# ExaScience/elprep

Measured on AMD Instinct MI355X. Metric: Mreads/s through sort+markdup+BQSR, 150bp PE, higher is better.
Workload: dtype u8/int32/int64 (integer path; float64 finalize on host)

## Files before the change

elprep_amd/csrc/markdup.hip:

```cpp
#include "common.hpp"
#include "markdup_plan.hpp"

namespace elp {

constexpr uint32_t EMPTY = 0xFFFFFFFFu;
constexpr unsigned long long PB_EMPTY = ~0ull;

struct MdCols {
  uint64_t n;
  const int32_t *refid;
  const uint16_t *flag_in;
  const uint16_t *rgid;
  const uint16_t *rg_lib;
  const uint16_t *split;
  const int32_t *upos, *score;
  const uint64_t *qname_off;
  const uint8_t *qname;
};

__device__ __forceinline__ bool is_candidate(uint16_t f) { return (f & (F_UNMAPPED | F_SECONDARY | F_SUPPLEMENTARY)) == 0; }
__device__ __forceinline__ bool is_true_pair(uint16_t f) { return (f & (F_MULTIPLE | F_NEXT_UNMAPPED)) == F_MULTIPLE; }
__device__ __forceinline__ uint16_t lib_of(const MdCols &m, uint32_t i) {
  const uint16_t rg = m.rgid[i];
  return rg == ELP_NIL16 ? (uint16_t)ELP_NIL16 : m.rg_lib[rg];
}
__device__ __forceinline__ uint32_t ld_agent(const uint32_t *p) { return __hip_atomic_load(p, __ATOMIC_RELAXED, __HIP_MEMORY_SCOPE_AGENT); }
__device__ __forceinline__ unsigned long long ld_agent64(const unsigned long long *p) {
  return __hip_atomic_load(p, __ATOMIC_RELAXED, __HIP_MEMORY_SCOPE_AGENT);
}

__device__ __forceinline__ bool key_eq(const uint4 &a, const uint4 &b) { return a.x == b.x && a.y == b.y && a.z == b.z && a.w == b.w; }
__device__ __forceinline__ uint64_t frag_hash(const uint4 &k) {
  const uint64_t h = ((uint64_t)k.x << 32) | k.y;
  return mix64(mix64(h) ^ (((uint64_t)k.w << 32) | (uint64_t)k.z));
}

template <class Eq>
__device__ __forceinline__ uint32_t find_or_insert(uint32_t *table, uint64_t mask, uint64_t h, uint32_t i, Eq eq, uint64_t limit = ~0ull) {
  uint64_t s = h & mask;
  for (uint64_t probes = 0;; probes++) {
    if (probes > limit) return EMPTY;
    const uint32_t cur = atomicCAS(&table[s], EMPTY, i);
    if (cur == EMPTY) return i;
    if (cur == i || eq(cur, i)) return cur;
    s = (s + 1) & mask;
  }
}

__global__ __launch_bounds__(256) void k_frag_insert(MdCols m, const uint4 *__restrict__ fkey, const uint32_t *__restrict__ flist, uint32_t nf,
                                                     uint32_t *table, uint64_t mask, uint32_t *__restrict__ frep, unsigned long long *fbest) {
  const uint32_t j = blockIdx.x * blockDim.x + threadIdx.x;
  if (j >= nf) return;
  const uint32_t i = flist[j];
  const uint4 mine = fkey[i];
  const uint32_t rep = find_or_insert(table, mask, frag_hash(mine), i, [&](uint32_t a, uint32_t) { return key_eq(fkey[a], mine); });
  frep[i] = rep;
  atomicMax(&fbest[rep], (unsigned long long)(uint32_t)m.score[i]);
}
__global__ __launch_bounds__(256) void k_frag_bits(const uint32_t *__restrict__ table, uint64_t nwords, uint32_t *__restrict__ bits) {
  const uint64_t w = (uint64_t)blockIdx.x * blockDim.x + threadIdx.x;
  if (w >= nwords) return;
  const uint4 *t = reinterpret_cast<const uint4 *>(table + 32 * w);
  uint32_t b = 0;
#pragma unroll
  for (int k = 0; k < 8; k++) {
    const uint4 v = t[k];
    b |= (v.x != EMPTY ? 1u : 0u) << (4 * k) | (v.y != EMPTY ? 2u : 0u) << (4 * k) | (v.z != EMPTY ? 4u : 0u) << (4 * k) | (v.w != EMPTY ? 8u : 0u) << (4 * k);
  }
  bits[w] = b;
}
__device__ __forceinline__ void tournament(const MdCols &m, uint32_t *winner, uint32_t me) {
  uint32_t w = ld_agent(winner);
  for (;;) {
    if (w == EMPTY) {
      const uint32_t old = atomicCAS(winner, EMPTY, me);
      if (old == EMPTY) return;
      w = old;
      continue;
    }
    const int cq = qname_cmp(m.qname, m.qname_off, me, w);
    const bool better = cq < 0 || (cq == 0 && me > w);
    if (!better) return;
    const uint32_t old = atomicCAS(winner, w, me);
    if (old == w) return;
    w = old;
  }
}

__global__ __launch_bounds__(256) void k_frag_tie(MdCols m, const uint32_t *__restrict__ flist, uint32_t nf, const uint32_t *__restrict__ frep,
                                                  const unsigned long long *__restrict__ fbest, uint32_t *fwinner) {
  const uint32_t j = blockIdx.x * blockDim.x + threadIdx.x;
  if (j >= nf) return;
  const uint32_t i = flist[j];
  const uint32_t rep = frep[i];
  const unsigned long long b = fbest[rep];
  if ((b >> 63) || (unsigned long long)(uint32_t)m.score[i] != b) return;
  tournament(m, &fwinner[rep], (uint32_t)i);
}

__global__ __launch_bounds__(256) void k_frag_flag(MdCols m, const uint32_t *__restrict__ flist, uint32_t nf, const uint32_t *__restrict__ frep,
                                                   const unsigned long long *__restrict__ fbest, const uint32_t *__restrict__ fwinner,
                                                   uint16_t *__restrict__ flag_out) {
  const uint32_t j = blockIdx.x * blockDim.x + threadIdx.x;
  if (j >= nf) return;
  const uint32_t i = flist[j];
  const uint32_t rep = frep[i];
  const unsigned long long b = fbest[rep];
  const bool dup = (b >> 63) || (unsigned long long)(uint32_t)m.score[i] < b || fwinner[rep] != (uint32_t)i;
  if (dup) flag_out[i] = (uint16_t)(flag_out[i] | F_DUPLICATE);
}

struct PairKey { uint4 k1, k2; };
__device__ __forceinline__ PairKey pair_key(const uint4 &second, const uint4 &first) {
  const int32_t r1 = (int32_t)second.x, r2 = (int32_t)first.x, p1 = (int32_t)second.y, p2 = (int32_t)first.y;
  const bool v1 = second.z & 1u, v2 = first.z & 1u;
  const bool swap = r1 > r2 || (r1 == r2 && (p1 > p2 || (p1 == p2 && v1 && !v2)));
  return swap ? PairKey{first, second} : PairKey{second, first};
}
__device__ __forceinline__ bool pair_key_eq(const PairKey &a, const PairKey &b) {
  return a.k1.x == b.k1.x && a.k2.x == b.k2.x && a.k1.y == b.k1.y && a.k2.y == b.k2.y && a.k1.z == b.k1.z && ((a.k2.z ^ b.k2.z) & 1u) == 0 &&
         a.k1.w == b.k1.w;
}

__device__ __forceinline__ uint64_t pair_hash(const PairKey &k) {
  uint64_t h = mix64(((uint64_t)k.k1.x << 32) | k.k2.x);
  h = mix64(h ^ (((uint64_t)k.k1.y << 32) | k.k2.y));
  return mix64(h ^ (((uint64_t)k.k1.z << 1) | (k.k2.z & 1u)) ^ ((uint64_t)k.k1.w << 40));
}

__device__ __forceinline__ uint64_t qname_hash(const MdCols &m, uint32_t i) {
  const uint64_t o = m.qname_off[i];
  const uint32_t l = (uint32_t)(m.qname_off[i + 1] - o);
  uint64_t h = 0x9e3779b97f4a7c15ull ^ l;
  for (uint32_t k = 0; k < l; k += 8) h = (h ^ low_bytes(load8(m.qname + o + k), l - k)) * 0xff51afd7ed558ccdull + (h >> 29);
  return mix64(h ^ ((uint64_t)lib_of(m, i) << 48) ^ ((uint64_t)m.split[i] << 24));
}
__device__ __forceinline__ bool mate_key_eq(const MdCols &m, const uint4 *__restrict__ fkey, uint32_t a, const uint4 &kb, uint32_t b) {
  const uint4 ka = fkey[a];
  return (ka.z >> 1) == (kb.z >> 1) && ka.w == kb.w && qname_eq(m.qname, m.qname_off, a, b);
}
__device__ __forceinline__ bool is_mate_candidate(uint16_t f) { return is_candidate(f) && is_true_pair(f); }

enum : uint8_t { MC_NONE = 0, MC_TABLE = 1, MC_LEAD = 2, MC_FOLLOW = 3, MC_KIND = 3, MC_TABBED = 4  };
constexpr uint32_t MATE_BIG = 0xFFFFFFFEu;

__global__ __launch_bounds__(256) void k_bloom_coarse(const uint32_t *__restrict__ bloom, uint32_t n_lines, uint32_t *__restrict__ coarse) {
  const uint32_t line = blockIdx.x * 256 + threadIdx.x;
  bool nz = false;
  if (line < n_lines) {
    const uint4 *l = reinterpret_cast<const uint4 *>(bloom + (size_t)line * 16);
    const uint4 a = l[0], b = l[1], c2 = l[2], d = l[3];
    nz = (a.x | a.y | a.z | a.w | b.x | b.y | b.z | b.w | c2.x | c2.y | c2.z | c2.w | d.x | d.y | d.z | d.w) != 0;
  }
  const unsigned long long bits = __ballot(nz);
// ... 132 lines not shown
  if (i >= n) return;
  const uint32_t r = rep_of[i];
  if (r == EMPTY) return;
  uint32_t rep;
  if (r == MATE_BIG) rep = (uint32_t)i;
  else if (rep_of[r] == MATE_BIG) rep = r;
  else return;
  const uint32_t at = atomicAdd(count, 1u);
  keys[at] = ((uint64_t)rep << 32) | (uint64_t)i;
  vals[at] = (uint32_t)i;
  mate[i] = EMPTY;
}
__global__ __launch_bounds__(256) void k_big_pair(uint32_t cnt, const uint64_t *__restrict__ keys, uint32_t *mate) {
  const uint32_t j = blockIdx.x * 256 + threadIdx.x;
  if (j >= cnt) return;
  const uint32_t rep = (uint32_t)(keys[j] >> 32);
  if (j > 0 && (uint32_t)(keys[j - 1] >> 32) == rep) return;
  for (uint32_t k = j; k + 1 < cnt && (uint32_t)(keys[k + 1] >> 32) == rep; k += 2) {
    const uint32_t a = (uint32_t)keys[k], b = (uint32_t)keys[k + 1];
    mate[a] = b;
    mate[b] = a;
  }
}

__device__ __forceinline__ uint64_t pair_entry(const MdCols &m, const uint4 &later, const uint4 &earlier, uint32_t i, uint32_t mt) {
  return ((uint64_t)(uint32_t)(m.score[i] + m.score[mt]) << 32) | (uint32_t)pair_hash(pair_key(later, earlier));
}
__global__ __launch_bounds__(256) void k_pair_list_table(MdCols m, const uint4 *__restrict__ fkey, const uint32_t *__restrict__ mate,
                                                         const uint8_t *__restrict__ code, uint64_t *__restrict__ pk, uint32_t *__restrict__ pv,
                                                         uint32_t *np) {
  __shared__ uint64_t lk[PL_TILES * 256];
  __shared__ uint32_t lv[PL_TILES * 256];
  __shared__ uint32_t lcount, gbase;
  if (threadIdx.x == 0) lcount = 0;
  __syncthreads();
#pragma unroll 2
  for (int tile = 0; tile < PL_TILES; tile++) {
    const uint64_t i64 = ((uint64_t)blockIdx.x * PL_TILES + (uint64_t)tile) * 256 + threadIdx.x;
    const uint32_t i = (uint32_t)i64;
    const uint32_t mt = (i64 < m.n && (code[i64] & MC_TABBED)) ? mate[i] : EMPTY;
    const bool own = mt != EMPTY && mt < i;
    uint64_t key = 0;
    if (own) key = pair_entry(m, fkey[i], fkey[mt], i, mt);
    const unsigned long long mask = __ballot(own);
    if (mask) {
      const int lane = threadIdx.x & 63, leader = __ffsll((long long)mask) - 1;
      uint32_t at = 0;
      if (lane == leader) at = atomicAdd(&lcount, (uint32_t)__popcll(mask));
      at = __shfl(at, leader, 64);
      if (own) {
        at += (uint32_t)__popcll(mask & ((1ull << lane) - 1ull));
        lk[at] = key;
        lv[at] = i;
      }
    }
  }
  __syncthreads();
  if (threadIdx.x == 0) gbase = lcount ? atomicAdd(np, lcount) : 0u;
  __syncthreads();
  for (uint32_t k = threadIdx.x; k < lcount; k += 256) {
    pk[gbase + k] = lk[k];
    pv[gbase + k] = lv[k];
  }
}

__global__ __launch_bounds__(256) void k_pair_list_lists(MdCols m, const uint4 *__restrict__ fkey, const uint32_t *__restrict__ mate, const uint32_t *__restrict__ tab_list,
                                                         const uint32_t *__restrict__ tab_cnt, uint32_t cap, uint64_t *__restrict__ pk, uint32_t *__restrict__ pv, uint32_t *np) {
  __shared__ uint32_t first[65];
  if (threadIdx.x < 64) {
    uint32_t incl = tab_cnt[threadIdx.x * 16u];
    for (int d = 1; d < 64; d <<= 1) {
      const uint32_t up = __shfl_up(incl, d, 64);
      if ((int)threadIdx.x >= d) incl += up;
    }
    first[threadIdx.x + 1] = incl;
    if (threadIdx.x == 0) first[0] = 0;
  }
  __syncthreads();
  __shared__ uint64_t lk[PL_TILES * 256];
  __shared__ uint32_t lv[PL_TILES * 256];
  __shared__ uint32_t lcount, gbase;
  const uint32_t total = first[64], chunk = PL_TILES * 256u;
  for (uint32_t c0 = blockIdx.x * chunk; c0 < total; c0 += gridDim.x * chunk) {
    if (threadIdx.x == 0) lcount = 0;
    __syncthreads();
#pragma unroll 2
    for (int tile = 0; tile < PL_TILES; tile++) {
      const uint32_t g = c0 + (uint32_t)tile * 256u + threadIdx.x;
      uint32_t i = 0, mt = EMPTY;
      if (g < total) {
        uint32_t lo = 0, hi = 64;
        while (hi - lo > 1) {
          const uint32_t mid = (lo + hi) >> 1;
          if (first[mid] <= g) lo = mid; else hi = mid;
        }
        i = tab_list[(size_t)lo * cap + (g - first[lo])];
        mt = mate[i];
      }
      const bool own = mt != EMPTY && mt < i;
      uint64_t key = 0;
      if (own) key = pair_entry(m, fkey[i], fkey[mt], i, mt);
      const unsigned long long mask = __ballot(own);
      if (mask) {
        const int lane = threadIdx.x & 63, leader = __ffsll((long long)mask) - 1;
        uint32_t at = 0;
        if (lane == leader) at = atomicAdd(&lcount, (uint32_t)__popcll(mask));
        at = __shfl(at, leader, 64);
        if (own) {
          at += (uint32_t)__popcll(mask & ((1ull << lane) - 1ull));
          lk[at] = key;
          lv[at] = i;
        }
      }
    }
    __syncthreads();
    if (threadIdx.x == 0) gbase = lcount ? atomicAdd(np, lcount) : 0u;
    __syncthreads();
    for (uint32_t k = threadIdx.x; k < lcount; k += 256) {
      pk[gbase + k] = lk[k];
      pv[gbase + k] = lv[k];
    }
    __syncthreads();
  }
}

__device__ __forceinline__ uint32_t pair_bucket(uint64_t key, int sbits, int bbits) {
  return bbits ? ((uint32_t)key & ((1u << sbits) - 1u)) >> (sbits - bbits) : 0u;
}
__global__ __launch_bounds__(256) void k_pair_bounds(const uint64_t *__restrict__ ks, const uint32_t *__restrict__ np, int sbits, int bbits,
                                                     uint32_t *__restrict__ bstart, uint32_t *__restrict__ bend) {
  const uint32_t n = *np;
  const uint32_t j = blockIdx.x * 256 + threadIdx.x;
  if (j >= n) return;
  const uint32_t b = pair_bucket(ks[j], sbits, bbits);
  if (j == 0 || pair_bucket(ks[j - 1], sbits, bbits) != b) bstart[b] = j;
  if (j + 1 == n || pair_bucket(ks[j + 1], sbits, bbits) != b) bend[b] = j + 1;
}

__device__ __forceinline__ PairKey pair_key_of(const uint4 *__restrict__ fkey, const uint32_t *__restrict__ mate, uint32_t owner) {
  return pair_key(fkey[owner], fkey[mate[owner]]);
}
__device__ __forceinline__ void tournament_lds(const MdCols &m, uint32_t *winner, uint32_t me) {
  uint32_t w = *(volatile uint32_t *)winner;
  for (;;) {
    if (w != EMPTY) {
      const int cq = qname_cmp(m.qname, m.qname_off, me, w);
      if (!(cq < 0 || (cq == 0 && me > w))) return;
    }
    const uint32_t old = atomicCAS(winner, w, me);
    if (old == w) return;
    w = old;
  }
}
__device__ __forceinline__ void pair_lost(const MdCols &m, const uint32_t *__restrict__ mate, uint32_t o, uint32_t w, uint32_t *__restrict__ pair_win,
                                          uint16_t *__restrict__ flag_out) {
  const uint32_t mt = mate[o];
  pair_win[o] = w;
  flag_out[o] = (uint16_t)(flag_out[o] | F_DUPLICATE);
  flag_out[mt] = (uint16_t)(flag_out[mt] | F_DUPLICATE);
}

constexpr int PB_ECAP = 1024;

__device__ __forceinline__ int pb_slot(const MdCols &m, const uint4 *__restrict__ fkey, const uint32_t *__restrict__ mate,
                                       unsigned long long *s_key, uint32_t tmask, uint32_t h32, uint32_t o, bool insert) {
  uint32_t idx = (h32 * 0x9E3779B1u) >> 16 & tmask;
  const unsigned long long mine = ((unsigned long long)h32 << 32) | o;
  for (uint32_t probes = 0; probes <= tmask; probes++, idx = (idx + 1) & tmask) {
    unsigned long long cur = insert ? atomicCAS(&s_key[idx], PB_EMPTY, mine) : s_key[idx];
    if (cur == PB_EMPTY) { if (insert) return (int)idx; else continue; }
    if (cur == mine) return (int)idx;
    if ((uint32_t)(cur >> 32) == h32 && pair_key_eq(pair_key_of(fkey, mate, (uint32_t)cur), pair_key_of(fkey, mate, o))) return (int)idx;
  }
  return -1;
}

__global__ __launch_bounds__(PB_THREADS) void k_pair_bucket(MdCols m, const uint4 *__restrict__ fkey, const uint32_t *__restrict__ mate,
                                                     const uint64_t *__restrict__ ks, uint32_t *__restrict__ vs,
                                                     const uint32_t *__restrict__ bstart, const uint32_t *__restrict__ bend, int cap_slots,
                                                     uint32_t *__restrict__ pair_win, uint16_t *__restrict__ flag_out, int inv_end ) {
  __shared__ unsigned long long s_key[PB_CAP];
  __shared__ uint32_t s_best[PB_CAP], s_win[PB_CAP];
  __shared__ uint16_t s_slot[PB_ECAP];
  __shared__ uint32_t s_full, s_min, s_h;
  const uint32_t start = bstart[blockIdx.x], end = inv_end ? ~bend[blockIdx.x] : bend[blockIdx.x];
  if (end <= start) return;
  const uint32_t cnt = end - start;
  const uint32_t t = threadIdx.x;
  if (cnt == 1) return;
  uint32_t T = 2;
  while (T < 2 * cnt && T < (uint32_t)cap_slots) T <<= 1;
  const uint32_t tmask = T - 1;
  for (uint32_t k = t; k < T; k += PB_THREADS) { s_key[k] = PB_EMPTY; s_best[k] = 0; s_win[k] = EMPTY; }
  if (t == 0) s_full = 0;
  __syncthreads();
  ks += start;
  vs += start;
  for (uint32_t e = t; e < cnt; e += PB_THREADS) {
    const uint64_t key = ks[e];
    const uint32_t o = vs[e];
    if (o == EMPTY) continue;
    const int slot = pb_slot(m, fkey, mate, s_key, tmask, (uint32_t)key, o, true);
    if (slot < 0) { s_full = 1; break; }
    atomicMax(&s_best[slot], (uint32_t)(key >> 32));
    if (e < PB_ECAP) s_slot[e] = (uint16_t)slot;
  }
  __syncthreads();
  if (!s_full) {
    for (uint32_t e = t; e < cnt; e += PB_THREADS) {
      const uint64_t key = ks[e];
      const uint32_t o = vs[e];
      if (o == EMPTY) continue;
      const int slot = e < PB_ECAP ? (int)s_slot[e] : pb_slot(m, fkey, mate, s_key, tmask, (uint32_t)key, o, false);
      if ((uint32_t)(key >> 32) == s_best[slot]) tournament_lds(m, &s_win[slot], o);
    }
    __syncthreads();
    for (uint32_t e = t; e < cnt; e += PB_THREADS) {
      const uint32_t o = vs[e];
      if (o == EMPTY) continue;
      const int slot = e < PB_ECAP ? (int)s_slot[e] : pb_slot(m, fkey, mate, s_key, tmask, (uint32_t)ks[e], o, false);
      const uint32_t w = s_win[slot];
      if (w != o) pair_lost(m, mate, o, w, pair_win, flag_out);
    }
    return;
  }
  for (;;) {
    __syncthreads();
    if (t == 0) { s_min = EMPTY; s_best[0] = 0; s_win[0] = EMPTY; }
    __syncthreads();
    for (uint32_t e = t; e < cnt; e += PB_THREADS) {
      const uint32_t o = vs[e];
      if (o != EMPTY) atomicMin(&s_min, o);
    }
    __syncthreads();
    const uint32_t rep = s_min;
    if (rep == EMPTY) return;
    for (uint32_t e = t; e < cnt; e += PB_THREADS)
      if (vs[e] == rep) s_h = (uint32_t)ks[e];
    __syncthreads();
    const uint32_t rh = s_h;
    const PairKey rk = pair_key_of(fkey, mate, rep);
    for (uint32_t e = t; e < cnt; e += PB_THREADS) {
      const uint32_t o = vs[e];
      if (o != EMPTY && (uint32_t)ks[e] == rh && pair_key_eq(rk, pair_key_of(fkey, mate, o))) atomicMax(&s_best[0], (uint32_t)(ks[e] >> 32));
    }
    __syncthreads();
    for (uint32_t e = t; e < cnt; e += PB_THREADS) {
      const uint32_t o = vs[e];
      if (o != EMPTY && (uint32_t)ks[e] == rh && (uint32_t)(ks[e] >> 32) == s_best[0] && pair_key_eq(rk, pair_key_of(fkey, mate, o)))
        tournament_lds(m, &s_win[0], o);
    }
    __syncthreads();
    for (uint32_t e = t; e < cnt; e += PB_THREADS) {
      const uint32_t o = vs[e];
      if (o != EMPTY && (uint32_t)ks[e] == rh && pair_key_eq(rk, pair_key_of(fkey, mate, o))) {
        if (s_win[0] != o) pair_lost(m, mate, o, s_win[0], pair_win, flag_out);
        vs[e] = EMPTY;
      }
    }
  }
}

__device__ __forceinline__ uint32_t next_lane(uint32_t x) { return (uint32_t)__builtin_amdgcn_update_dpp(0, (int)x, 0x130 , 0xf, 0xf, false); }
__device__ __forceinline__ uint64_t next_lane64(uint64_t x) { return (uint64_t)next_lane((uint32_t)x) | ((uint64_t)next_lane((uint32_t)(x >> 32)) << 32); }

struct FrontCols {
  uint64_t n;
  const int32_t *refid, *pos;
  const uint16_t *flag;
  const uint8_t *state;
  const uint16_t *rgid, *rg_lib, *split;
  const uint64_t *cigar_off;
  const uint32_t *cigar;
  const uint64_t *qname_off;
  const uint8_t *qname;
  uint32_t n_ref;
  int pos_bits;
};
__device__ __forceinline__ int32_t unclipped_pos(uint16_t f, int32_t p, uint64_t c0, uint64_t c1, const uint32_t *__restrict__ cigar, uint32_t o0, uint32_t o1,
                                                 uint32_t o2, uint32_t o3) {
  if ((f & (F_UNMAPPED | F_SECONDARY | F_SUPPLEMENTARY)) != 0) return 0;
  int32_t up = p;
  const uint64_t nop = c1 - c0;
  auto at = [&](uint64_t k) __attribute__((always_inline)) -> uint32_t { return k == 0 ? o0 : (k == 1 ? o1 : (k == 2 ? o2 : (k == 3 ? o3 : cigar[c0 + k]))); };
  if (nop) {
    if (f & F_REVERSED) {
      int32_t clipped = 1;
      up--;
      for (uint64_t k = nop; k-- > 0;) {
        const uint32_t c = at(k), op = c & 0xF;
        const int32_t isclip = (op == OP_S || op == OP_H) ? 1 : 0;
        const int32_t isref = op_consumes_ref(op) ? 1 : 0;
        clipped *= isclip;
        up += (isref | clipped) * (int32_t)(c >> 4);
      }
    } else {
      for (uint64_t k = 0; k < nop; k++) {
        const uint32_t c = at(k), op = c & 0xF;
        if (!(op == OP_S || op == OP_H)) break;
        up -= (int32_t)(c >> 4);
      }
    }
  }
  return up;
}
__device__ __forceinline__ uint16_t flag_in_of(uint16_t f, uint8_t state) { return state == 2 ? (uint16_t)(f | F_SECONDARY) : f; }

constexpr int FLI_CAP = 4096;
__global__ __launch_bounds__(256) void k_frag_list(FrontCols m, uint4 *__restrict__ fkey, uint32_t *__restrict__ flist, uint32_t *nf,
                                                   unsigned long long *__restrict__ fbest, uint32_t *__restrict__ fwinner) {
  __shared__ uint32_t lq[FLI_CAP];
  __shared__ uint32_t lcount, gbase;
  if (threadIdx.x == 0) lcount = 0;
  __syncthreads();
  const uint64_t nchunks = (m.n + FLI_CHUNK - 1) / FLI_CHUNK;
  for (uint64_t ch = blockIdx.x; ch < nchunks; ch += gridDim.x) {
    const uint64_t i0 = (ch * 256 + threadIdx.x) * 8;
    uint4 fv = make_uint4(0, 0, 0, 0);
    uint2 sv = make_uint2(0, 0);
    if (i0 < m.n) {
      fv = *reinterpret_cast<const uint4 *>(m.flag + i0);
      sv = *reinterpret_cast<const uint2 *>(m.state + i0);
    }
    const uint32_t fw[4] = {fv.x, fv.y, fv.z, fv.w};
    const uint64_t st8 = (uint64_t)sv.x | ((uint64_t)sv.y << 32);
    uint32_t fm = 0;
#pragma unroll
    for (int k = 0; k < 8; k++) {
      const uint16_t f = flag_in_of((uint16_t)(fw[k >> 1] >> (16 * (k & 1))), (uint8_t)(st8 >> (8 * k)));
      if (i0 + (uint64_t)k < m.n && is_candidate(f) && !is_true_pair(f)) fm |= 1u << k;
    }
    if (fm) {
      uint32_t at = atomicAdd(&lcount, (uint32_t)__popc(fm));
      for (; fm; fm &= fm - 1u) lq[at++] = (uint32_t)i0 + (uint32_t)(__ffs((int)fm) - 1);
    }
    __syncthreads();
    const uint32_t cnt = lcount;
    if (cnt + FLI_CHUNK <= (uint32_t)FLI_CAP && ch + gridDim.x < nchunks) continue;
    if (threadIdx.x == 0) gbase = cnt ? atomicAdd(nf, cnt) : 0u;
    __syncthreads();
    for (uint32_t k = threadIdx.x; k < cnt; k += 256) {
      const uint32_t i = lq[k];
      const uint16_t f = m.flag[i], rg = m.rgid[i];
      const uint64_t c0 = m.cigar_off[i], c1 = m.cigar_off[i + 1];
      const uint64_t nop = c1 - c0;
      const uint32_t o0 = nop > 0 ? m.cigar[c0] : 0u, o1 = nop > 1 ? m.cigar[c0 + 1] : 0u, o2 = nop > 2 ? m.cigar[c0 + 2] : 0u, o3 = nop > 3 ? m.cigar[c0 + 3] : 0u;
      const uint16_t lib = rg == ELP_NIL16 ? (uint16_t)ELP_NIL16 : m.rg_lib[rg];
      const int32_t up = unclipped_pos(f, m.pos[i], c0, c1, m.cigar, o0, o1, o2, o3);
      fkey[i] = make_uint4((uint32_t)m.refid[i], (uint32_t)up, ((uint32_t)lib << 1) | ((f & F_REVERSED) ? 1u : 0u), (uint32_t)m.split[i]);
      fbest[i] = 0;
      fwinner[i] = EMPTY;
      flist[gbase + k] = i;
    }
    __syncthreads();
    if (threadIdx.x == 0) lcount = 0;
    __syncthreads();
  }
}

template <bool ADAPT>
__global__ __launch_bounds__(MF_THREADS) void k_md_front(FrontCols m, const int32_t *__restrict__ score, int32_t *__restrict__ upos_out, uint64_t *__restrict__ key_out,
                                                         uint4 *fkey, uint8_t *__restrict__ code, uint32_t *__restrict__ hash32, uint32_t *__restrict__ hash_lo, uint32_t *bloom,
                                                         uint32_t bloom_mask, uint32_t *n_table, const uint32_t *__restrict__ ftable, const uint32_t *__restrict__ fbits,
                                                         uint64_t fmask , unsigned long long *fbest, uint32_t *__restrict__ mate,
                                                         uint32_t *__restrict__ pair_win, uint64_t *__restrict__ pk, uint32_t *__restrict__ pv, uint32_t *np,
                                                         uint32_t nfixed, int optimistic) {
  const uint64_t base = (uint64_t)blockIdx.x * MF_RECS;
  const uint32_t t = threadIdx.x, lane = t & 63u, u = 63u * (t >> 6) + lane;
  const int64_t a_s = (int64_t)base - 2 + (int64_t)u;
  const bool own_rec = a_s >= 0 && (uint64_t)a_s < m.n;
  const bool valid = a_s >= 0 && (uint64_t)a_s + 1 < m.n;
  const uint64_t a = own_rec ? (uint64_t)a_s : 0;
  const uint16_t fa_st = m.flag[a], ra = m.rgid[a], sa = m.split[a];
  const uint8_t sta = m.state[a];
  const int32_t r = m.refid[a], p = m.pos[a], sc = score[a];
  const uint64_t oa = m.qname_off[a], oa1 = m.qname_off[a + 1];
  const uint64_t c0 = m.cigar_off[a], c1 = m.cigar_off[a + 1];
  const uint32_t la = (uint32_t)(oa1 - oa);
  const uint64_t nop = c1 - c0;
  const uint16_t lia = ra == ELP_NIL16 ? (uint16_t)ELP_NIL16 : m.rg_lib[ra];
  const uint8_t *pa = m.qname + oa;
  const uint64_t a0 = load8(pa), a1 = load8(pa + 8), a2 = load8(pa + 16), a3 = load8(pa + 24);
  const uint32_t o0 = nop > 0 ? m.cigar[c0] : 0u, o1 = nop > 1 ? m.cigar[c0 + 1] : 0u, o2 = nop > 2 ? m.cigar[c0 + 2] : 0u, o3 = nop > 3 ? m.cigar[c0 + 3] : 0u;
  const uint16_t fa = flag_in_of(fa_st, sta);
  const int32_t up = unclipped_pos(fa_st, p, c0, c1, m.cigar, o0, o1, o2, o3);
  const uint4 mine = make_uint4((uint32_t)r, (uint32_t)up, ((uint32_t)lia << 1) | ((fa & F_REVERSED) ? 1u : 0u), (uint32_t)sa);
  const uint64_t w0 = la > 0 ? low_bytes(a0, la) : 0ull, w1 = la > 8 ? low_bytes(a1, la - 8) : 0ull, w2 = la > 16 ? low_bytes(a2, la - 16) : 0ull,
                 w3 = la > 24 ? low_bytes(a3, la - 24) : 0ull;
  const uint32_t mcand = own_rec && is_mate_candidate(fa) ? 1u : 0u;
  const uint32_t nA = next_lane(mcand | ((uint32_t)lia << 1)), nL = next_lane(la);
  const uint32_t nS = next_lane((uint32_t)sa);
  const uint64_t b0 = next_lane64(w0), b1 = next_lane64(w1), b2 = next_lane64(w2), b3 = next_lane64(w3);
  const uint64_t n_oa = next_lane64(oa);
  bool join = valid && lane < 63u && mcand && (nA & 1u) && (uint16_t)(nA >> 1) == lia && (uint16_t)nS == sa && nL == la;
  if (join) {
    join = ((w0 ^ b0) | (w1 ^ b1) | (w2 ^ b2) | (w3 ^ b3)) == 0;
    const uint8_t *pb = m.qname + n_oa;
    for (uint32_t k = 32; join && k < la; k += 8) join = low_bytes(load8(pa + k), la - k) == low_bytes(load8(pb + k), la - k);
  }
  __shared__ uint8_t s_join[320];
  __shared__ uint4 s_fk[316];
  __shared__ int32_t s_sc[316];
  if (lane < 63u) {
    s_join[u] = join;
    s_fk[u] = mine;
    s_sc[u] = sc;
  }
  __syncthreads();
  const bool mine_rec = own_rec && lane < 63u && u >= 2u && u < 2u + (uint32_t)MF_RECS;
// ... 59 lines not shown
struct MdBufs {
  MdCols m;
  uint32_t *table, *rep, *flist, *winner, *bloom, *coarse, *hash32, *tab_list, *hash_lo;
  unsigned long long *best;
  uint4 *fkey;
  uint8_t *code;
  uint64_t *pk;
  uint32_t *pv, *ftable, *fbits;
  uint32_t *nf_dev, *np_dev, *n_table_dev;
  uint32_t *rep_of;
};
constexpr size_t MD_CTRS = 16 + 64 * 16;

static int md_carve(elp_ctx *c, const MdScratch &L, MdBufs *b) {
  b->m = MdCols{c->n, c->refid.p, c->flag.p, c->rgid.p, c->rg_lib.p, c->split.p, c->upos.p, c->score.p, c->qname_off.p, c->qname.p};
  ELP_TRY(scratch(c, 0, L.table, &b->table));
  ELP_TRY(scratch(c, 2, L.best, &b->best));
  ELP_TRY(scratch(c, 3, L.winner, &b->winner));
  ELP_TRY(scratch(c, 5, L.fkey, &b->fkey));
  ELP_TRY(ensure(c, c->md_ctr, MD_CTRS));
  ELP_TRY(scratch(c, 1, L.words1, &b->rep));
  b->flist = b->rep + L.flist;
  b->nf_dev = c->md_ctr.p, b->np_dev = c->md_ctr.p + 1, b->n_table_dev = c->md_ctr.p + 16;
  b->rep_of = c->pair_win.p;
  return 0;
}

static int md_frag_list(elp_ctx *c, const MdSizes &S, const MdBufs &B, const FrontCols &fc) {
  hipStream_t st = c->stream;
  ELP_HIP(c, hipMemsetAsync(c->md_ctr.p, 0, MD_CTRS * sizeof(uint32_t), st));
  ELP_TRY(mailbox(c));
  ELP_LAUNCH(c, "md_frag_list", k_frag_list, dim3(S.frag_list_grid(c->n_cu)), dim3(256), 0, fc, B.fkey, B.flist, B.nf_dev, B.best, B.winner);
  ELP_HIP(c, hipMemcpyAsync(c->mail, B.nf_dev, 4, hipMemcpyDeviceToHost, st));
  ELP_HIP(c, hipEventRecord(c->mail_ev, st));
  return 0;
}

static int md_front(elp_ctx *c, const MdSizes &S, const MdScratch &L, MdBufs &B, const FrontCols &fc, bool fuse_adapt, uint32_t *nf_out) {
  hipStream_t st = c->stream;
  ELP_TRY(scratch(c, 6, L.words6, &B.bloom));
  B.coarse = B.bloom + L.coarse, B.hash32 = B.bloom + L.hash32, B.tab_list = B.bloom + L.tab_list, B.hash_lo = B.bloom + L.hash_lo;
  B.code = reinterpret_cast<uint8_t *>(B.bloom + L.code);
  ELP_HIP(c, hipMemsetAsync(B.bloom, 0, S.bw * sizeof(uint32_t), st));
  ELP_HIP(c, elp::event_wait(c->mail_ev));
  const uint32_t nf = *nf_out = c->mail[0];
  const uint64_t Tf = frag_table_size(nf, S.T);
  const MdScratch::Pairs P = L.pairs(Tf);
  ELP_TRY(scratch(c, 7, P.words64, &B.pk));
  uint32_t *const w7 = reinterpret_cast<uint32_t *>(B.pk);
  B.pv = w7 + P.pv, B.ftable = w7 + P.ftable, B.fbits = w7 + P.fbits;
  if (nf) {
    ELP_HIP(c, hipMemsetAsync(B.ftable, 0xFF, Tf * sizeof(uint32_t), st));
    ELP_LAUNCH(c, "md_frag_insert", k_frag_insert, dim3(blocks_for(nf, 256)), dim3(256), 0, B.m, (const uint4 *)B.fkey, (const uint32_t *)B.flist, nf, B.ftable, Tf - 1, B.rep, B.best);
    ELP_LAUNCH(c, "md_frag_bits", k_frag_bits, dim3(blocks_for(Tf / 32, 256)), dim3(256), 0, (const uint32_t *)B.ftable, Tf / 32, B.fbits);
  }
  const auto front = fuse_adapt ? k_md_front<true> : k_md_front<false>;
  ELP_LAUNCH(c, "md_front", front, dim3(S.front_grid), dim3(MF_THREADS), 0, fc, (const int32_t *)c->score.p, c->upos.p, c->key.p, B.fkey, B.code, B.hash32, B.hash_lo, B.bloom,
             (uint32_t)(S.bw - 1), B.n_table_dev, (const uint32_t *)B.ftable, (const uint32_t *)B.fbits, nf ? Tf - 1 : (uint64_t)0, B.best, c->mate.p, c->pair_win.p, B.pk, B.pv, B.np_dev, S.nfx,
             c->tune.mate_path == 0 ? 1 : 0);
  return 0;
}

static int md_fragments(elp_ctx *c, const MdBufs &B, uint32_t nf, uint32_t *n_tab_out) {
  hipStream_t st = c->stream;
  if (nf) {
    const unsigned fgrid = blocks_for(nf, 256);
    ELP_LAUNCH(c, "md_frag_tie", k_frag_tie, dim3(fgrid), dim3(256), 0, B.m, (const uint32_t *)B.flist, nf, (const uint32_t *)B.rep, (const unsigned long long *)B.best, B.winner);
    ELP_LAUNCH(c, "md_frag_flag", k_frag_flag, dim3(fgrid), dim3(256), 0, B.m, (const uint32_t *)B.flist, nf, (const uint32_t *)B.rep, (const unsigned long long *)B.best,
               (const uint32_t *)B.winner, c->flag.p);
  }
  uint32_t n_tab64[64 * 16], adapt_word[ADAPT_WORDS] = {0, 0, 0, 0, 0, 0};
  ELP_HIP(c, hipMemcpyAsync(n_tab64, B.n_table_dev, sizeof n_tab64, hipMemcpyDeviceToHost, st));
  const bool adapt_read = c->derived.adapt_pending;
  if (adapt_read) ELP_HIP(c, hipMemcpyAsync(adapt_word, c->adapt_err.p, sizeof adapt_word, hipMemcpyDeviceToHost, st));
  ELP_HIP(c, elp::stream_wait(st));
  if (adapt_read) adapt_note(c, adapt_word);
  if (c->derived.adapt_bad_qual) return adapt_quality_error(c);
  *n_tab_out = 0;
  for (int k = 0; k < 64; k++) *n_tab_out += n_tab64[k * 16];
  return 0;
}

static int md_mates(elp_ctx *c, const MdSizes &S, const MdBufs &B, const MatePlan &P, uint32_t n_tab, bool *big) {
  hipStream_t st = c->stream;
  const uint64_t n = S.n;
  ELP_HIP(c, hipMemsetAsync(c->mate.p, 0xFF, n * sizeof(uint32_t), st));
  if (n_tab) ELP_LAUNCH(c, "md_bloom_coarse", k_bloom_coarse, dim3(S.coarse_grid), dim3(256), 0, (const uint32_t *)B.bloom, (uint32_t)(S.bw / 16), B.coarse);
  uint32_t e[4] = {0, 0, 0, 0};
  for (uint64_t Tm = P.Tm;; Tm = S.T) {
    ELP_HIP(c, hipMemsetAsync(B.table, 0xFF, Tm * sizeof(uint32_t), st));
    ELP_HIP(c, hipMemsetD32Async(reinterpret_cast<hipDeviceptr_t>(B.np_dev), (int)(uint32_t)P.nfixed, 1, st));
    if (P.listed) ELP_HIP(c, hipMemsetAsync(B.n_table_dev, 0, 64 * 16 * sizeof(uint32_t), st));
    ELP_LAUNCH(c, "md_mate_pairs", k_mate_pairs, dim3(S.mate_grid), dim3(256), 0, B.m, (const uint4 *)B.fkey, B.code, (const uint32_t *)B.hash32, (const uint32_t *)B.hash_lo,
               (const uint32_t *)B.bloom, (uint32_t)(S.bw - 1), (const uint32_t *)(n_tab ? B.coarse : nullptr), B.table, Tm - 1, c->mate.p, B.rep_of, c->err_flag.p, P.fixed ? 1 : 0, B.pk,
               B.pv, P.listed ? B.tab_list : (uint32_t *)nullptr, B.n_table_dev, S.tab_cap);
    if (P.listed)
      ELP_LAUNCH(c, "md_mate_table", k_mate_table, dim3(blocks_for(P.list_n, 256)), dim3(256), 0, B.m, (const uint4 *)B.fkey, (const uint8_t *)B.code, (const uint32_t *)B.hash32,
                 (const uint32_t *)B.hash_lo, (const uint32_t *)B.tab_list, (const uint32_t *)B.n_table_dev, S.tab_cap, B.table, Tm - 1, c->mate.p, B.rep_of, c->err_flag.p);
    ELP_TRY(fetch_err(c, e));
    if (!(e[1] & 2u)) break;
    if (Tm == S.T) return set_error(c, ELP_ERR_HIP, "mark duplicates: mate table overflow");
    ELP_HIP(c, hipMemsetAsync(c->err_flag.p + 1, 0, 4, st));
    ELP_HIP(c, hipMemsetAsync(c->mate.p, 0xFF, n * sizeof(uint32_t), st));
    ELP_HIP(c, hipMemsetAsync(B.rep_of, 0xFF, n * sizeof(uint32_t), st));
  }
  *big = e[1] != 0;
  return 0;
}

static int md_big_groups(elp_ctx *c, const MdSizes &S, const MdScratch &L, const MdBufs &B) {
  hipStream_t st = c->stream;
  ELP_HIP(c, hipMemsetAsync(c->err_flag.p + 1, 0, 4, st));
  uint64_t *bk, *ks;
  uint32_t *bv, *vs, *cnt_dev = c->err_flag.p + 3;
  ELP_TRY(scratch(c, 2, L.big, &bk));
  ELP_TRY(scratch(c, 3, L.big, &bv));
  ELP_HIP(c, hipMemsetAsync(cnt_dev, 0, 4, st));
  ELP_LAUNCH(c, "md_big_collect", k_big_collect, dim3(S.grid), dim3(256), 0, S.n, (const uint32_t *)B.rep_of, c->mate.p, bk, bv, cnt_dev);
  uint32_t cnt = 0;
  ELP_HIP(c, hipMemcpyAsync(&cnt, cnt_dev, 4, hipMemcpyDeviceToHost, st));
  ELP_HIP(c, elp::stream_wait(st));
  ELP_HIP(c, hipMemsetAsync(cnt_dev, 0, 4, st));
  ProfScope ps(c, "md_big_");
  ELP_TRY(radix_sort_pairs(c, bk, bv, bk + S.n, bv + S.n, cnt, &ks, &vs));
  ELP_LAUNCH(c, "md_big_pair", k_big_pair, dim3(blocks_for(cnt, 256)), dim3(256), 0, cnt, (const uint64_t *)ks, c->mate.p);
  return 0;
}

static int md_pairs(elp_ctx *c, const MdSizes &S, const MdScratch &L, const MdBufs &B, const MatePlan &P) {
  hipStream_t st = c->stream;
  uint32_t *bounds;
  ELP_TRY(scratch(c, 1, L.bounds_words, &bounds));
  const bool folded = S.ndig > 0;
  ELP_HIP(c, hipMemsetAsync(bounds, folded ? 0xFF : 0, 2 * S.nb * sizeof(uint32_t), st));
  if (!P.fast) {
    ELP_HIP(c, hipMemsetAsync(c->pair_win.p, 0xFF, S.n * sizeof(uint32_t), st));
    if (P.listed)
      ELP_LAUNCH(c, "md_pair_list", k_pair_list_lists, dim3(blocks_for(P.list_n, 256 * PL_TILES)), dim3(256), 0, B.m, (const uint4 *)B.fkey, (const uint32_t *)c->mate.p, (const uint32_t *)B.tab_list,
                 (const uint32_t *)B.n_table_dev, S.tab_cap, B.pk, B.pv, B.np_dev);
    else
      ELP_LAUNCH(c, "md_pair_list", k_pair_list_table, dim3(S.list_grid), dim3(256), 0, B.m, (const uint4 *)B.fkey, (const uint32_t *)c->mate.p, (const uint8_t *)B.code, B.pk, B.pv,
                 B.np_dev);
  }
  uint64_t *ks = B.pk;
  uint32_t *vs = B.pv;
  if (folded) {
    ProfScope ps(c, "md_pair_");
    ELP_TRY(radix_sort_pairs_low(c, B.pk, B.pv, B.pk + S.npmax, B.pv + S.npmax, S.npmax, S.ndig, &ks, &vs, nullptr, false, B.np_dev,
                                 RadixBounds{bounds, bounds + S.nb, (uint32_t)((1ull << S.sbits) - 1ull), S.sbits - S.bbits}));
  } else {
    ELP_LAUNCH(c, "md_pair_bounds", k_pair_bounds, dim3(S.bounds_grid), dim3(256), 0, (const uint64_t *)ks, (const uint32_t *)B.np_dev, S.sbits, S.bbits, bounds, bounds + S.nb);
  }
  ELP_LAUNCH(c, "md_pair_bucket", k_pair_bucket, dim3((unsigned)S.nb), dim3(PB_THREADS), 0, B.m, (const uint4 *)B.fkey, (const uint32_t *)c->mate.p, (const uint64_t *)ks, vs,
             (const uint32_t *)bounds, (const uint32_t *)(bounds + S.nb), std::min(c->tune.pair_table_slots, PB_CAP), c->pair_win.p, c->flag.p, folded ? 1 : 0);
  return 0;
}

static int markdup_impl(elp_ctx *c) {
  const uint64_t n = c->n;
  ELP_TRY(ensure(c, c->mate, n + 1));
  ELP_TRY(ensure(c, c->pair_win, n + 1));
  if (n == 0) { ELP_TRY(ensure_adapted(c, true)); c->derived.marked = true; return 0; }
  const bool fuse_adapt = !c->derived.adapted();
  int pos_bits = 1;
  if (fuse_adapt) ELP_TRY(adapt_begin(c, &pos_bits));
  else ELP_TRY(ensure_adapted(c, false));
  const MdSizes S(n);
  const MdScratch L(S);
  MdBufs B;
  ELP_TRY(md_carve(c, L, &B));
  const FrontCols fc{n, c->refid.p, c->pos.p, c->flag.p, c->has_sr.p, c->rgid.p, c->rg_lib.p, c->split.p, c->cigar_off.p, c->cigar.p, c->qname_off.p, c->qname.p,
                     (uint32_t)c->n_ref, pos_bits};
  ELP_TRY(md_frag_list(c, S, B, fc));
  if (fuse_adapt) ELP_TRY(adapt_scores(c));
  uint32_t nf = 0, n_tab = 0;
  ELP_TRY(md_front(c, S, L, B, fc, fuse_adapt, &nf));
  if (fuse_adapt) c->derived.keys = c->derived.scores = true;
  ELP_TRY(sort_presort(c));
  ELP_TRY(md_fragments(c, B, nf, &n_tab));
  const MatePlan P = mate_plan(n, n_tab, c->tune.mate_path, S.T);
  bool big = false;
  if (!P.fast) ELP_TRY(md_mates(c, S, B, P, n_tab, &big));
  if (big) ELP_TRY(md_big_groups(c, S, L, B));
  ELP_TRY(md_pairs(c, S, L, B, P));
  c->radix_check_pending = true;
  c->derived.marked = true;
  return 0;
}

}

extern "C" int elp_mark_duplicates(elp_ctx *c, int also_opticals) {
  (void)also_opticals;
  if (!c) return ELP_ERR_ARG;
  ELP_HIP(c, hipSetDevice(c->device));
  c->derived.drop_marked();
  return elp::markdup_impl(c);
}
```

elprep_amd/csrc/markdup_plan.hpp:

```cpp
#pragma once
#include <algorithm>
#include <cstddef>
#include <cstdint>

namespace elp {

constexpr int MP_R = 1;
constexpr int PL_TILES = 8;
constexpr int PB_THREADS = 256;
constexpr int PB_TARGET = 384;
constexpr int PB_CAP = 1024;
constexpr int FLI_CHUNK = 2048;
constexpr int MF_THREADS = 320, MF_RECS = 312;

inline unsigned md_blocks(uint64_t n, unsigned per_block) { return (unsigned)((n + per_block - 1) / per_block); }

inline uint64_t table_size_for(uint64_t n) {
  uint64_t t = 1024;
  while (t < 2 * n + 16) t <<= 1;
  return t;
}

struct MdSizes {
  uint64_t n, T;
  int bbits, ndig, sbits;
  size_t nb;
  uint64_t bw;
  uint32_t tab_cap;
  uint64_t npmax;
  uint32_t nfx;
  unsigned grid, frag_list_blocks, front_grid, mate_grid, coarse_grid, list_grid, bounds_grid;
  explicit MdSizes(uint64_t records) : n(records), T(table_size_for(records)), bbits(0), bw(1024), npmax(records + 2), nfx((uint32_t)((records + 1) / 2)) {
    while (bbits < 24 && ((n / 2 + 1) >> bbits) > (uint64_t)PB_TARGET) bbits++;
    ndig = (bbits + 7) / 8;
    sbits = 8 * ndig;
    nb = (size_t)1 << bbits;
    while (bw < n / 16 && bw < (1u << 20)) bw <<= 1;
    grid = md_blocks(n, 256);
    frag_list_blocks = md_blocks(n, FLI_CHUNK);
    front_grid = md_blocks(n, MF_RECS);
    mate_grid = md_blocks(n, 256 * MP_R);
    coarse_grid = md_blocks(bw / 16, 256);
    list_grid = md_blocks(n, 256 * PL_TILES);
    bounds_grid = md_blocks(npmax, 256);
    tab_cap = (uint32_t)((mate_grid + 63) / 64) * 256u * MP_R;
  }
  unsigned frag_list_grid(int n_cu) const { return std::min<unsigned>(frag_list_blocks, (unsigned)n_cu * 8); }
};

struct MdScratch {
  size_t table, best, winner, fkey, big;
  size_t flist, words1, bounds_words;
  size_t coarse, hash32, code, tab_list, hash_lo, words6;
  uint64_t npmax;
  explicit MdScratch(const MdSizes &s) : npmax(s.npmax) {
    const size_t n = (size_t)s.n;
    table = (size_t)s.T;
    best = winner = n + 16;
    fkey = n + 8;
    big = 2 * n + 8;
    flist = n + 8;
    words1 = flist + n + 8;
    bounds_words = 2 * s.nb + 8;
    coarse = (size_t)s.bw;
    hash32 = coarse + (size_t)s.bw / 512 + 16;
    code = hash32 + n + 8;
    tab_list = code + 8 + (n + 16) / 4;
    hash_lo = tab_list + 64 * (size_t)s.tab_cap + 8;
    words6 = hash_lo + 8 + n + 16;
  }
  struct Pairs { size_t pv, ftable, fbits, words64; };
  Pairs pairs(uint64_t Tf) const {
    const size_t pv = 4 * (size_t)npmax, ftable = pv + 2 * (size_t)npmax, fbits = ftable + (size_t)Tf;
    return Pairs{pv, ftable, fbits, (fbits + (size_t)Tf / 32 + 64) / 2 + 8};
  }
};

inline uint64_t frag_table_size(uint32_t nf, uint64_t T) { return nf ? std::min<uint64_t>(T, table_size_for(4ull * nf)) : 0; }

struct MatePlan {
  bool fixed, fast, listed;
  uint64_t nfixed, Tm, list_n;
};
inline MatePlan mate_plan(uint64_t n, uint32_t n_tab, int mate_path, uint64_t T) {
  const bool fixed = (uint64_t)n_tab < n / 8 && mate_path == 0;
  return MatePlan{fixed, fixed && n_tab == 0, fixed && n_tab != 0, fixed ? (n + 1) / 2 : 0,
                  fixed ? std::min<uint64_t>(T, table_size_for(std::min<uint64_t>(n, 4ull * n_tab + 1024))) : T, std::min<uint64_t>(n, 2ull * n_tab + 4096)};
}

}
```

Measured before the change: 2475.

## Restructure pair-bucket markdup kernel with register-resident entries and batched hash collision settling

```diff
diff --git a/elprep_amd/csrc/markdup.hip b/elprep_amd/csrc/markdup.hip
--- a/elprep_amd/csrc/markdup.hip
+++ b/elprep_amd/csrc/markdup.hip
@@ -1,5 +1,6 @@
 #include "common.hpp"
 #include "markdup_plan.hpp"
+#include <utility>
 
 namespace elp {
 
@@ -438,109 +439,216 @@
     w = old;
   }
 }
-__device__ __forceinline__ void pair_lost(const MdCols &m, const uint32_t *__restrict__ mate, uint32_t o, uint32_t w, uint32_t *__restrict__ pair_win,
-                                          uint16_t *__restrict__ flag_out) {
-  const uint32_t mt = mate[o];
+__device__ __forceinline__ void flag_or(uint32_t *__restrict__ flag_words, uint32_t word, uint32_t bits) {
+  (void)__hip_atomic_fetch_or(flag_words + word, bits, __ATOMIC_RELAXED, __HIP_MEMORY_SCOPE_AGENT);
+}
+__device__ __forceinline__ void pair_lost(uint32_t o, uint32_t mt, uint32_t w, uint32_t *__restrict__ pair_win, uint32_t *__restrict__ flag_words) {
   pair_win[o] = w;
-  flag_out[o] = (uint16_t)(flag_out[o] | F_DUPLICATE);
-  flag_out[mt] = (uint16_t)(flag_out[mt] | F_DUPLICATE);
-}
-
-constexpr int PB_ECAP = 1024;
-
-__device__ __forceinline__ int pb_slot(const MdCols &m, const uint4 *__restrict__ fkey, const uint32_t *__restrict__ mate,
-                                       unsigned long long *s_key, uint32_t tmask, uint32_t h32, uint32_t o, bool insert) {
-  uint32_t idx = (h32 * 0x9E3779B1u) >> 16 & tmask;
+  const uint32_t bo = (uint32_t)F_DUPLICATE << (16u * (o & 1u)), bm = (uint32_t)F_DUPLICATE << (16u * (mt & 1u));
+  if ((o >> 1) == (mt >> 1)) flag_or(flag_words, o >> 1, bo | bm);
+  else { flag_or(flag_words, o >> 1, bo); flag_or(flag_words, mt >> 1, bm); }
+}
+
+constexpr uint32_t PB_PEND = 0x80000000u, PB_FULL = 0x40000000u, PB_SLOT = 0xFFFFu;
+constexpr uint32_t PB_QUEUED = 0x20000000u, PB_TIED = 0x10000000u;
+__device__ __forceinline__ uint32_t pb_home(uint32_t h32, uint32_t tmask) { return (h32 * 0x9E3779B1u) >> 16 & tmask; }
+__device__ __forceinline__ uint32_t pb_probe(unsigned long long *s_key, uint32_t tmask, uint32_t h32, uint32_t o, uint32_t skip) {
+  const uint32_t home = pb_home(h32, tmask);
   const unsigned long long mine = ((unsigned long long)h32 << 32) | o;
-  for (uint32_t probes = 0; probes <= tmask; probes++, idx = (idx + 1) & tmask) {
-    unsigned long long cur = insert ? atomicCAS(&s_key[idx], PB_EMPTY, mine) : s_key[idx];
-    if (cur == PB_EMPTY) { if (insert) return (int)idx; else continue; }
-    if (cur == mine) return (int)idx;
-    if ((uint32_t)(cur >> 32) == h32 && pair_key_eq(pair_key_of(fkey, mate, (uint32_t)cur), pair_key_of(fkey, mate, o))) return (int)idx;
-  }
-  return -1;
-}
+  for (uint32_t p = skip; p <= tmask; p++) {
+    const uint32_t idx = (home + p) & tmask;
+    const unsigned long long cur = atomicCAS(&s_key[idx], PB_EMPTY, mine);
+    if (cur == PB_EMPTY || cur == mine) return idx;
+    if ((uint32_t)(cur >> 32) == h32) return idx | PB_PEND;
+  }
+  return PB_FULL;
+}
+__device__ __forceinline__ uint32_t pb_settle(const uint4 *__restrict__ fkey, const uint32_t *__restrict__ mate, unsigned long long *s_key, uint32_t tmask,
+                                              uint32_t s, uint32_t o, uint32_t mt, uint32_t mc) {
+  const PairKey mine = pair_key(fkey[o], fkey[mt]);
+  for (;;) {
+    const uint32_t idx = s & PB_SLOT;
+    const unsigned long long cur = s_key[idx];
+    if (pair_key_eq(pair_key(fkey[(uint32_t)cur], fkey[mc]), mine)) return idx;
+    const uint32_t h32 = (uint32_t)(cur >> 32);
+    s = pb_probe(s_key, tmask, h32, o, ((idx - pb_home(h32, tmask)) & tmask) + 1u);
+    if (!(s & PB_PEND)) return s;
+    mc = mate[(uint32_t)s_key[s & PB_SLOT]];
+  }
+}
+__device__ __forceinline__ uint32_t pb_slot(const uint4 *__restrict__ fkey, const uint32_t *__restrict__ mate, unsigned long long *s_key, uint32_t tmask,
+                                            uint32_t h32, uint32_t o) {
+  const uint32_t s = pb_probe(s_key, tmask, h32, o, 0);
+  return (s & PB_PEND) ? pb_settle(fkey, mate, s_key, tmask, s, o, mate[o], mate[(uint32_t)s_key[s & PB_SLOT]]) : s;
+}
+template <class F, int... R>
+__device__ __forceinline__ void pb_each_(F &&f, std::integer_sequence<int, R...>) { (f(std::integral_constant<int, R>{}), ...); }
+template <class F>
+__device__ __forceinline__ void pb_each(F &&f) { pb_each_(f, std::make_integer_sequence<int, PB_R>{}); }
 
 __global__ __launch_bounds__(PB_THREADS) void k_pair_bucket(MdCols m, const uint4 *__restrict__ fkey, const uint32_t *__restrict__ mate,
                                                      const uint64_t *__restrict__ ks, uint32_t *__restrict__ vs,
                                                      const uint32_t *__restrict__ bstart, const uint32_t *__restrict__ bend, int cap_slots,
-                                                     uint32_t *__restrict__ pair_win, uint16_t *__restrict__ flag_out, int inv_end ) {
+                                                     uint32_t *__restrict__ pair_win, uint32_t *__restrict__ flag_words, int inv_end ) {
   __shared__ unsigned long long s_key[PB_CAP];
   __shared__ uint32_t s_best[PB_CAP], s_win[PB_CAP];
-  __shared__ uint16_t s_slot[PB_ECAP];
-  __shared__ uint32_t s_full, s_min, s_h;
+  __shared__ uint2 s_q[PB_THREADS];
+  __shared__ uint32_t s_ctl[4];
   const uint32_t start = bstart[blockIdx.x], end = inv_end ? ~bend[blockIdx.x] : bend[blockIdx.x];
   if (end <= start) return;
   const uint32_t cnt = end - start;
   const uint32_t t = threadIdx.x;
   if (cnt == 1) return;
-  uint32_t T = 2;
-  while (T < 2 * cnt && T < (uint32_t)cap_slots) T <<= 1;
-  const uint32_t tmask = T - 1;
-  for (uint32_t k = t; k < T; k += PB_THREADS) { s_key[k] = PB_EMPTY; s_best[k] = 0; s_win[k] = EMPTY; }
-  if (t == 0) s_full = 0;
-  __syncthreads();
   ks += start;
   vs += start;
-  for (uint32_t e = t; e < cnt; e += PB_THREADS) {
+  uint32_t sc[PB_R], hs[PB_R], o[PB_R];
+  pb_each([&](auto R) {
+    constexpr int r = R;
+    const uint32_t e = pb_entry(t, r);
+    sc[r] = hs[r] = 0;
+    o[r] = EMPTY;
+    if (e < cnt) {
+      const uint64_t key = ks[e];
+      o[r] = vs[e];
+      hs[r] = o[r] != EMPTY ? (uint32_t)key : 0u;
+      sc[r] = (uint32_t)(key >> 32);
+    }
+  });
+  const uint32_t T = pb_table_slots(cnt, (uint32_t)cap_slots), tmask = T - 1;
+  for (uint32_t k = t; k < T; k += PB_THREADS) { s_key[k] = PB_EMPTY; s_best[k] = 0; s_win[k] = EMPTY; }
+  if (t == 0) s_ctl[0] = s_ctl[3] = 0;
+  __syncthreads();
+  uint32_t mt[PB_R];
+  pb_each([&](auto R) {
+    constexpr int r = R;
+    mt[r] = EMPTY;
+    if (o[r] != EMPTY) hs[r] = pb_probe(s_key, tmask, hs[r], o[r], 0);
+  });
+  for (;;) {
+    pb_each([&](auto R) {
+      constexpr int r = R;
+      if (hs[r] & PB_PEND) {
+        const uint32_t at = atomicAdd(&s_ctl[3], 1u);
+        if (at < (uint32_t)PB_THREADS) {
+          s_q[at] = make_uint2(o[r], hs[r] & PB_SLOT);
+          hs[r] = PB_QUEUED | at;
+        }
+      }
+    });
+    __syncthreads();
+    const uint32_t asked = *(volatile uint32_t *)&s_ctl[3];
+    if (asked == 0) break;
+    if (t < asked) {
+      const uint2 it = s_q[t];
+      const uint32_t mo = mate[it.x], mc = mate[(uint32_t)s_key[it.y]];
+      s_q[t] = make_uint2(pb_settle(fkey, mate, s_key, tmask, it.y | PB_PEND, it.x, mo, mc), mo);
+    }
+    __syncthreads();
+    pb_each([&](auto R) {
+      constexpr int r = R;
+      if (hs[r] & PB_QUEUED) {
+        const uint2 res = s_q[hs[r] & PB_SLOT];
+        hs[r] = res.x;
+        mt[r] = res.y;
+      }
+    });
+    if (asked <= (uint32_t)PB_THREADS) break;
+    __syncthreads();
+    if (t == 0) s_ctl[3] = 0;
+    __syncthreads();
+  }
+  pb_each([&](auto R) {
+    constexpr int r = R;
+    if (o[r] != EMPTY) {
+      if (hs[r] == PB_FULL) s_ctl[0] = 1;
+      else atomicMax(&s_best[hs[r]], sc[r]);
+    }
+  });
+  for (uint32_t e = t + PB_ECAP; e < cnt; e += PB_THREADS) {
     const uint64_t key = ks[e];
-    const uint32_t o = vs[e];
-    if (o == EMPTY) continue;
-    const int slot = pb_slot(m, fkey, mate, s_key, tmask, (uint32_t)key, o, true);
-    if (slot < 0) { s_full = 1; break; }
+    const uint32_t oe = vs[e];
+    if (oe == EMPTY) continue;
+    const uint32_t slot = pb_slot(fkey, mate, s_key, tmask, (uint32_t)key, oe);
+    if (slot == PB_FULL) { s_ctl[0] = 1; break; }
     atomicMax(&s_best[slot], (uint32_t)(key >> 32));
-    if (e < PB_ECAP) s_slot[e] = (uint16_t)slot;
   }
   __syncthreads();
-  if (!s_full) {
+  if (!*(volatile uint32_t *)&s_ctl[0]) {
+    pb_each([&](auto R) {
+      constexpr int r = R;
+      if (o[r] != EMPTY && sc[r] == s_best[hs[r]] && atomicCAS(&s_win[hs[r]], EMPTY, o[r]) != EMPTY) hs[r] |= PB_TIED;
+    });
+    for (;;) {
+      uint32_t me = EMPTY, slot = 0;
+      pb_each([&](auto R) {
+        constexpr int r = R;
+        if (hs[r] & PB_TIED) { me = o[r]; slot = hs[r] & PB_SLOT; }
+      });
+      if (me == EMPTY) break;
+      pb_each([&](auto R) {
+        constexpr int r = R;
+        if (o[r] == me) hs[r] = slot;
+      });
+      tournament_lds(m, &s_win[slot], me);
+    }
+    for (uint32_t e = t + PB_ECAP; e < cnt; e += PB_THREADS) {
+      const uint64_t key = ks[e];
+      const uint32_t oe = vs[e];
+      if (oe == EMPTY) continue;
+      const uint32_t slot = pb_slot(fkey, mate, s_key, tmask, (uint32_t)key, oe);
+      if ((uint32_t)(key >> 32) == s_best[slot]) tournament_lds(m, &s_win[slot], oe);
+    }
+    __syncthreads();
+    pb_each([&](auto R) {
+      constexpr int r = R;
+      sc[r] = EMPTY;
+      if (o[r] != EMPTY) sc[r] = *(volatile uint32_t *)&s_win[hs[r]];
+      if (sc[r] != o[r] && mt[r] == EMPTY) mt[r] = mate[o[r]];
+    });
+    pb_each([&](auto R) {
+      constexpr int r = R;
+      if (sc[r] != o[r]) pair_lost(o[r], mt[r], sc[r], pair_win, flag_words);
+    });
+    for (uint32_t e = t + PB_ECAP; e < cnt; e += PB_THREADS) {
+      const uint32_t oe = vs[e];
+      if (oe == EMPTY) continue;
+      const uint32_t w = *(volatile uint32_t *)&s_win[pb_slot(fkey, mate, s_key, tmask, (uint32_t)ks[e], oe)];
+      if (w != oe) pair_lost(oe, mate[oe], w, pair_win, flag_words);
+    }
+    return;
+  }
+  for (;;) {
+    __syncthreads();
+    if (t == 0) { s_ctl[1] = EMPTY; s_best[0] = 0; s_win[0] = EMPTY; }
+    __syncthreads();
     for (uint32_t e = t; e < cnt; e += PB_THREADS) {
-      const uint64_t key = ks[e];
-      const uint32_t o = vs[e];
-      if (o == EMPTY) continue;
-      const int slot = e < PB_ECAP ? (int)s_slot[e] : pb_slot(m, fkey, mate, s_key, tmask, (uint32_t)key, o, false);
-      if ((uint32_t)(key >> 32) == s_best[slot]) tournament_lds(m, &s_win[slot], o);
-    }
-    __syncthreads();
-    for (uint32_t e = t; e < cnt; e += PB_THREADS) {
-      const uint32_t o = vs[e];
-      if (o == EMPTY) continue;
-      const int slot = e < PB_ECAP ? (int)s_slot[e] : pb_slot(m, fkey, mate, s_key, tmask, (uint32_t)ks[e], o, false);
-      const uint32_t w = s_win[slot];
-      if (w != o) pair_lost(m, mate, o, w, pair_win, flag_out);
-    }
-    return;
-  }
-  for (;;) {
-    __syncthreads();
-    if (t == 0) { s_min = EMPTY; s_best[0] = 0; s_win[0] = EMPTY; }
-    __syncthreads();
-    for (uint32_t e = t; e < cnt; e += PB_THREADS) {
-      const uint32_t o = vs[e];
-      if (o != EMPTY) atomicMin(&s_min, o);
-    }
-    __syncthreads();
-    const uint32_t rep = s_min;
+      const uint32_t oe = vs[e];
+      if (oe != EMPTY) atomicMin(&s_ctl[1], oe);
+    }
+    __syncthreads();
+    const uint32_t rep = *(volatile uint32_t *)&s_ctl[1];
     if (rep == EMPTY) return;
     for (uint32_t e = t; e < cnt; e += PB_THREADS)
-      if (vs[e] == rep) s_h = (uint32_t)ks[e];
-    __syncthreads();
-    const uint32_t rh = s_h;
+      if (vs[e] == rep) s_ctl[2] = (uint32_t)ks[e];
+    __syncthreads();
+    const uint32_t rh = *(volatile uint32_t *)&s_ctl[2];
     const PairKey rk = pair_key_of(fkey, mate, rep);
     for (uint32_t e = t; e < cnt; e += PB_THREADS) {
-      const uint32_t o = vs[e];
-      if (o != EMPTY && (uint32_t)ks[e] == rh && pair_key_eq(rk, pair_key_of(fkey, mate, o))) atomicMax(&s_best[0], (uint32_t)(ks[e] >> 32));
+      const uint32_t oe = vs[e];
+      if (oe != EMPTY && (uint32_t)ks[e] == rh && pair_key_eq(rk, pair_key_of(fkey, mate, oe))) atomicMax(&s_best[0], (uint32_t)(ks[e] >> 32));
     }
     __syncthreads();
     for (uint32_t e = t; e < cnt; e += PB_THREADS) {
-      const uint32_t o = vs[e];
-      if (o != EMPTY && (uint32_t)ks[e] == rh && (uint32_t)(ks[e] >> 32) == s_best[0] && pair_key_eq(rk, pair_key_of(fkey, mate, o)))
-        tournament_lds(m, &s_win[0], o);
+      const uint32_t oe = vs[e];
+      if (oe != EMPTY && (uint32_t)ks[e] == rh && (uint32_t)(ks[e] >> 32) == *(volatile uint32_t *)&s_best[0] && pair_key_eq(rk, pair_key_of(fkey, mate, oe)))
+        tournament_lds(m, &s_win[0], oe);
     }
     __syncthreads();
     for (uint32_t e = t; e < cnt; e += PB_THREADS) {
-      const uint32_t o = vs[e];
-      if (o != EMPTY && (uint32_t)ks[e] == rh && pair_key_eq(rk, pair_key_of(fkey, mate, o))) {
-        if (s_win[0] != o) pair_lost(m, mate, o, s_win[0], pair_win, flag_out);
+      const uint32_t oe = vs[e];
+      if (oe != EMPTY && (uint32_t)ks[e] == rh && pair_key_eq(rk, pair_key_of(fkey, mate, oe))) {
+        const uint32_t w = *(volatile uint32_t *)&s_win[0];
+        if (w != oe) pair_lost(oe, mate[oe], w, pair_win, flag_words);
         vs[e] = EMPTY;
       }
     }
@@ -906,7 +1014,8 @@
     ELP_LAUNCH(c, "md_pair_bounds", k_pair_bounds, dim3(S.bounds_grid), dim3(256), 0, (const uint64_t *)ks, (const uint32_t *)B.np_dev, S.sbits, S.bbits, bounds, bounds + S.nb);
   }
   ELP_LAUNCH(c, "md_pair_bucket", k_pair_bucket, dim3((unsigned)S.nb), dim3(PB_THREADS), 0, B.m, (const uint4 *)B.fkey, (const uint32_t *)c->mate.p, (const uint64_t *)ks, vs,
-             (const uint32_t *)bounds, (const uint32_t *)(bounds + S.nb), std::min(c->tune.pair_table_slots, PB_CAP), c->pair_win.p, c->flag.p, folded ? 1 : 0);
+             (const uint32_t *)bounds, (const uint32_t *)(bounds + S.nb), std::min(c->tune.pair_table_slots, PB_CAP), c->pair_win.p,
+             reinterpret_cast<uint32_t *>(c->flag.p), folded ? 1 : 0);
   return 0;
 }
 
diff --git a/elprep_amd/csrc/markdup_plan.hpp b/elprep_amd/csrc/markdup_plan.hpp
--- a/elprep_amd/csrc/markdup_plan.hpp
+++ b/elprep_amd/csrc/markdup_plan.hpp
@@ -7,9 +7,11 @@
 
 constexpr int MP_R = 1;
 constexpr int PL_TILES = 8;
-constexpr int PB_THREADS = 256;
+constexpr int PB_THREADS = 128;
 constexpr int PB_TARGET = 384;
-constexpr int PB_CAP = 1024;
+constexpr int PB_CAP = 512;
+constexpr int PB_ECAP = 512;
+constexpr int PB_R = PB_ECAP / PB_THREADS;
 constexpr int FLI_CHUNK = 2048;
 constexpr int MF_THREADS = 320, MF_RECS = 312;
 
@@ -47,6 +49,15 @@
   }
   unsigned frag_list_grid(int n_cu) const { return std::min<unsigned>(frag_list_blocks, (unsigned)n_cu * 8); }
 };
+
+constexpr uint32_t pb_table_slots(uint32_t cnt, uint32_t cap) {
+  uint32_t T = 2;
+  while ((uint64_t)T < 2 * (uint64_t)cnt && T < cap) T <<= 1;
+  return T;
+}
+constexpr uint32_t pb_entry(uint32_t t, int r) { return t + (uint32_t)r * PB_THREADS; }
+static_assert(PB_THREADS % 64 == 0 && PB_ECAP % PB_THREADS == 0, "whole waves, every register slot of every thread used");
+static_assert((PB_CAP & (PB_CAP - 1)) == 0 && PB_CAP >= 4 && PB_CAP <= 65536, "table slots: a power of two whose indices fit 16 bits");
 
 struct MdScratch {
   size_t table, best, winner, fkey, big;
```

Measured after the change: 2484 (median of 2 runs). About the same (+0.3%).
